# auniquesun/PPT

Measured on AMD Instinct MI355X. Metric: point-clouds/sec fwd+bwd, PointBERT 1024-pt ModelNet40, higher is better.
Workload: dtype f16; 1 GPU; C2: ModelNet40 1024-pt PointBERT (ULIP_PointBERT head_type=0, frozen backbone + PromptLearner), train-mode BN + DropPath, fwd + CE(ls 0.2) + bwd + AdamW; feed=resident, per_gpu_batch=32, global_batch=32, npoints=1024, classes=40, parallelism=dp1

## Files before the change

### include/ppt_hip.h

```cpp
#ifndef PPT_HIP_H
#define PPT_HIP_H

#include <stddef.h>
#include <stdint.h>

#ifdef __cplusplus
extern "C" {
#endif

#define PPT_OK 0
#define PPT_EINVAL (-1)
#define PPT_ELAUNCH (-2)
#define PPT_EUNSUPPORTED (-3)

#define PPT_F32 0
#define PPT_BF16 1
#define PPT_F16 2

const char *ppt_strerror(int code);
int ppt_abi_version(void);

int ppt_fps_f32(const float *xyz, int B, int N, int M, const int64_t *start, int64_t *out_idx,
                float *out_xyz, void *stream);

// ... 181 lines not shown
    int wave_prio;
} ppt_text_lin_params;
int ppt_text_lin_retile_split(const float *W, void *W_tiled, int N, int K, int b_pow2, void *stream);
int ppt_text_lin_split(const ppt_text_lin_params *p, void *stream);
typedef struct ppt_text_lin16_params {
    const void *A; int64_t lda;
    const void *W;
    const float *bias;
    const float *residual; int64_t ld_res;
    void *C; int64_t ldc;
    int M, N, K;
    int dtype;
    int c_dtype;
    int wave_prio;
} ppt_text_lin16_params;
int ppt_text_lin_retile16(const void *W, void *W_tiled, int N, int K, void *stream);
int ppt_text_lin16(const ppt_text_lin16_params *p, void *stream);

int ppt_attention_fwd(const void *qkv, void *out, float *lse, int Bt, int T, int H, int hd,
                      float scale, int causal, int dtype, void *stream);
int ppt_attention_bwd(const void *qkv, const void *out, const void *dout, const float *lse,
                      float *delta, void *dqkv, int Bt, int T, int H, int hd, float scale,
                      int causal, int dtype, void *stream);

size_t ppt_attention_prefix_workspace_bytes(int C, int P, int H, int hd);
int ppt_attention_fwd_split16(const void *qkv, void *out, float *lse, int Bt, int T, int P, int H, int hd, float scale, int causal,
                              void *stream);
int ppt_attention_bwd_split16(const void *qkv, const void *out, const void *dout, const float *lse, float *delta, void *dqkv,
                              float *workspace, int Bt, int T, int P, int H, int hd, float scale, int causal, void *stream);
int ppt_attention_prefix_fwd(const void *qkv, void *out, float *lse, int C, int T, int P, int H, int hd, float scale, int dtype,
                             void *stream);
int ppt_attention_prefix_bwd(const void *qkv, const void *out, const void *dout, const float *lse, float *delta, void *dqkv,
                             float *workspace, int C, int T, int P, int H, int hd, float scale, int dtype, void *stream);

int ppt_conv1_stats(const float *pts, int64_t M, const float *w1, const float *b1, int C,
                    float *part_sum, float *part_sqsum, int *n_partials, void *stream);
int ppt_bn_finalize(const float *part_sum, const float *part_sqsum, int n_partials,
                    int rows_per_partial, int64_t count, int C, const float *gamma, const float *beta, float eps, int train,
                    float momentum, float *running_mean, float *running_var,
                    int64_t *num_batches_tracked, float *scale, float *shift, void *stream);
size_t ppt_bn_finalize_workspace_bytes(int n_partials, int C);
int ppt_bn_finalize_ws(const float *part_sum, const float *part_sqsum, int n_partials,
                       int rows_per_partial, int64_t count, int C, const float *gamma, const float *beta, float eps, int train,
                       float momentum, float *running_mean, float *running_var,
                       int64_t *num_batches_tracked, float *scale, float *shift,
                       float *mean_out , float *rstd_out ,
                       void *workspace, size_t workspace_bytes, void *stream);

int ppt_rows_stats_rows_per_partial(void);
int ppt_rows_stats_f32(const float *x, int64_t M, int C, float *part_sum, float *part_m2, void *stream);
int ppt_bn_rows_bwd_reduce(const float *dy, const float *x, const float *scale, const float *shift, const float *mean,
                           const float *rstd, int relu, int64_t M, int C, float *part_g, float *part_gx, void *stream);
int ppt_bn_rows_bwd_apply(const float *dy, const float *x, const float *scale, const float *shift, const float *mean,
                          const float *rstd, const float *sum_g, const float *sum_gx, int relu, int batch_stats, int64_t M,
                          int C, float *dx, void *dx_half, int half_dtype, void *stream);
int ppt_conv1_stats_max_partials(int64_t M);
int ppt_conv1_stats_rows_per_partial(void);

int ppt_gn_stats_chunks(int R);
int ppt_gn_bwd_chunks(int Q);
int ppt_gn_finish(const double *part, int B, int nch, int G, double n, double eps, int mode, float *out0, float *out1, void *stream);
int ppt_gn_stats(const float *y, int B, int R, int C, int G, double *part, void *stream);
int ppt_gn_lrelu_max(const float *y, const float *mean, const float *rstd, const float *gamma, const float *beta, int B, int Q, int K,
                     int C, int G, float slope, float *out, int32_t *arg, void *stream);
int ppt_gn_bwd_sums(const float *y, const float *dout, const float *out, const int32_t *arg, const float *mean, const float *rstd,
                    const float *gamma, int B, int Q, int K, int C, int G, float slope, double *psum, float *pgb, void *stream);
// ... 114 lines not shown
```

### ppt_amd/_lib.py

```python
import ctypes
import os

_HERE = os.path.dirname(os.path.abspath(__file__))
LIB_PATH = os.environ.get("PPT_HIP_LIB") or os.path.join(_HERE, "csrc", "libppt_hip.so")
_lib = None

PPT_F32, PPT_BF16, PPT_F16 = 0, 1, 2
A_PLAIN, A_AFFINE_RELU, A_CONV1 = 0, 1, 2
ACT_NONE, ACT_RELU, ACT_GELU, ACT_QUICKGELU = 0, 1, 2, 3

c_void_p, c_int, c_int64, c_float, c_size_t = (ctypes.c_void_p, ctypes.c_int, ctypes.c_int64,
                                               ctypes.c_float, ctypes.c_size_t)


class GemmParams(ctypes.Structure):
    _fields_ = [
        ("A", c_void_p), ("lda", c_int64), ("B", c_void_p), ("ldb", c_int64),
        ("C", c_void_p), ("ldc", c_int64), ("M", c_int), ("N", c_int), ("K", c_int),
        ("dtype", c_int), ("c_dtype", c_int),
        ("a_mode", c_int), ("a_scale", c_void_p), ("a_shift", c_void_p), ("pts", c_void_p),
        ("w1", c_void_p), ("b1", c_void_p),
        ("bias", c_void_p), ("group_add", c_void_p), ("group_rows", c_int), ("act", c_int),
        ("dact_pre", c_void_p), ("ld_dact", c_int64),
        ("row_scale", c_void_p), ("row_scale_rows", c_int),
        ("residual", c_void_p), ("ld_res", c_int64), ("residual2", c_void_p), ("ld_res2", c_int64),
        ("C2", c_void_p), ("ldc2", c_int64), ("c2_dtype", c_int), ("c2_pre", c_int),
        ("col_sum", c_void_p), ("col_sqsum", c_void_p), ("pool_max", c_void_p), ("pool_dtype", c_int), ("pool_rows", c_int), ("pool_min", c_void_p),
        ("batch", c_int), ("strideA", c_int64), ("strideB", c_int64), ("strideC", c_int64), ("wave_prio", c_int),
        ("split16", c_int), ("split_a_pow2", c_int), ("split_b_pow2", c_int), ("split_overflow", c_void_p),
    ]


class LnLinParams(ctypes.Structure):
    _fields_ = [
        ("x", c_void_p), ("W", c_void_p), ("C", c_void_p), ("ln_w", c_void_p), ("ln_b", c_void_p), ("ln_eps", ctypes.c_float),
        ("bias", c_void_p), ("M", c_int), ("N", c_int), ("K", c_int), ("dtype", c_int), ("slices", c_int),
    ]


class TextLinParams(ctypes.Structure):
# ... 87 lines not shown
    "ppt_lnlin_retile": (c_int, [c_void_p, c_void_p, c_int, c_void_p]),
    "ppt_lnlin": (c_int, [ctypes.POINTER(LnLinParams), c_void_p]),
    "ppt_text_mlp_retile": (c_int, [c_void_p, c_void_p, c_void_p, c_void_p, c_void_p]),
    "ppt_text_mlp_pair": (c_int, [ctypes.POINTER(TextMlpParams), c_void_p]),
    "ppt_text_mlp_retile_split": (c_int, [c_void_p, c_void_p, c_void_p, c_void_p, c_int, c_void_p]),
    "ppt_text_lin_retile_split": (c_int, [c_void_p, c_void_p, c_int, c_int, c_int, c_void_p]),
    "ppt_text_lin_split": (c_int, [ctypes.POINTER(TextLinParams), c_void_p]),
    "ppt_text_lin_retile16": (c_int, [c_void_p, c_void_p, c_int, c_int, c_void_p]),
    "ppt_text_lin16": (c_int, [ctypes.POINTER(TextLin16Params), c_void_p]),
    "ppt_vit_mlp3_retile": (c_int, [c_void_p, c_void_p, c_void_p, c_void_p, c_void_p]),
    "ppt_vit_mlp3_bf16": (c_int, [ctypes.POINTER(VitMlpParams), c_void_p]),
    "ppt_rowgemm_bf16": (c_int, [ctypes.POINTER(RowGemmParams), c_void_p]),
    "ppt_layernorm_fwd": (c_int, [c_void_p, c_void_p, c_int, c_void_p, c_void_p, c_void_p, c_void_p, c_int,
                                  c_void_p, c_void_p, c_int, c_int, c_float, c_void_p]),
    "ppt_layernorm_bwd": (c_int, [c_void_p, c_void_p, c_void_p, c_void_p, c_void_p, c_void_p, c_int,
                                  c_void_p, c_int, c_void_p, c_void_p, c_int, c_int, c_int, c_void_p]),
    "ppt_layernorm_fwd_sum": (c_int, [c_void_p, c_void_p, c_void_p, c_int, c_void_p, c_void_p, c_void_p, c_void_p, c_int,
                                      c_void_p, c_void_p, c_int, c_int, c_float, c_void_p]),
    "ppt_layernorm_bwd_sum": (c_int, [c_void_p, c_int, c_void_p, c_void_p, c_void_p, c_void_p, c_void_p, c_int,
                                      c_void_p, c_int, c_int, c_int, c_void_p]),
    "ppt_col_sums": (c_int, [c_void_p, c_int, c_int, c_int, c_int64, c_void_p, c_void_p]),
    "ppt_attention_fwd": (c_int, [c_void_p, c_void_p, c_void_p, c_int, c_int, c_int, c_int, c_float, c_int,
                                  c_int, c_void_p]),
    "ppt_attention_bwd": (c_int, [c_void_p, c_void_p, c_void_p, c_void_p, c_void_p, c_void_p, c_int, c_int,
                                  c_int, c_int, c_float, c_int, c_int, c_void_p]),
    "ppt_attention_prefix_workspace_bytes": (ctypes.c_size_t, [c_int, c_int, c_int, c_int]),
    "ppt_pointmlp_cloud_rstd": (c_int, [c_void_p, c_int, c_int, ctypes.c_double, c_void_p, c_void_p]),
    "ppt_pointmlp_pq": (c_int, [c_void_p, c_void_p, c_void_p, c_void_p, c_void_p, c_void_p, c_int, c_int, c_int, c_int, c_void_p]),
    "ppt_attention_bwd_split16": (c_int, [c_void_p, c_void_p, c_void_p, c_void_p, c_void_p, c_void_p, c_void_p, c_int, c_int, c_int, c_int, c_int, c_float, c_int, c_void_p]),
    "ppt_attention_fwd_split16": (c_int, [c_void_p, c_void_p, c_void_p, c_int, c_int, c_int, c_int, c_int, c_float, c_int, c_void_p]),
    "ppt_attention_prefix_fwd": (c_int, [c_void_p, c_void_p, c_void_p, c_int, c_int, c_int, c_int, c_int, c_float, c_int, c_void_p]),
    "ppt_attention_prefix_bwd": (c_int, [c_void_p, c_void_p, c_void_p, c_void_p, c_void_p, c_void_p, c_void_p, c_int, c_int, c_int,
                                         c_int, c_int, c_float, c_int, c_void_p]),
    "ppt_conv1_stats": (c_int, [c_void_p, c_int64, c_void_p, c_void_p, c_int, c_void_p, c_void_p,
                                ctypes.POINTER(c_int), c_void_p]),
    "ppt_conv1_stats_max_partials": (c_int, [c_int64]),
    "ppt_conv1_stats_rows_per_partial": (c_int, []),
    "ppt_bn_finalize": (c_int, [c_void_p, c_void_p, c_int, c_int, c_int64, c_int, c_void_p, c_void_p, c_float, c_int,
                                c_float, c_void_p, c_void_p, c_void_p, c_void_p, c_void_p, c_void_p]),
    "ppt_bn_finalize_ws": (c_int, [c_void_p, c_void_p, c_int, c_int, c_int64, c_int, c_void_p, c_void_p, c_float, c_int,
                                   c_float, c_void_p, c_void_p, c_void_p, c_void_p, c_void_p, c_void_p, c_void_p, c_void_p,
                                   ctypes.c_size_t, c_void_p]),
    "ppt_rows_stats_rows_per_partial": (c_int, []),
    "ppt_rows_stats_f32": (c_int, [c_void_p, c_int64, c_int, c_void_p, c_void_p, c_void_p]),
    "ppt_bn_rows_bwd_reduce": (c_int, [c_void_p, c_void_p, c_void_p, c_void_p, c_void_p, c_void_p, c_int, c_int64, c_int,
                                       c_void_p, c_void_p, c_void_p]),
    "ppt_bn_rows_bwd_apply": (c_int, [c_void_p, c_void_p, c_void_p, c_void_p, c_void_p, c_void_p, c_void_p, c_void_p, c_int,
                                      c_int, c_int64, c_int, c_void_p, c_void_p, c_int, c_void_p]),
    "ppt_bn_finalize_workspace_bytes": (ctypes.c_size_t, [c_int, c_int]),
    "ppt_gn_stats_chunks": (c_int, [c_int]),
    "ppt_gn_bwd_chunks": (c_int, [c_int]),
    "ppt_gn_stats": (c_int, [c_void_p, c_int, c_int, c_int, c_int, c_void_p, c_void_p]),
    "ppt_gn_lrelu_max": (c_int, [c_void_p, c_void_p, c_void_p, c_void_p, c_void_p, c_int, c_int, c_int, c_int, c_int, c_float,
                                 c_void_p, c_void_p, c_void_p]),
    "ppt_gn_bwd_sums": (c_int, [c_void_p, c_void_p, c_void_p, c_void_p, c_void_p, c_void_p, c_void_p, c_int, c_int, c_int, c_int,
                                c_int, c_float, c_void_p, c_void_p, c_void_p]),
    "ppt_gn_bwd_apply": (c_int, [c_void_p, c_void_p, c_void_p, c_void_p, c_void_p, c_void_p, c_void_p, c_void_p, c_int, c_int,
                                 c_int, c_int, c_int, c_float, c_void_p, c_void_p]),
    "ppt_mini_pointnet_conv12_bf16": (c_int, [c_void_p, c_int64, c_void_p, c_void_p, c_void_p, c_void_p, c_int, c_void_p, c_void_p,
                                              c_int, c_void_p, c_void_p, c_void_p]),
    "ppt_mini_pointnet_conv3_bf16": (c_int, [c_void_p, c_int64, c_int, c_void_p, c_void_p, c_int, c_void_p, c_void_p, c_void_p,
                                             c_void_p]),
    "ppt_mini_pointnet_conv4_bf16": (c_int, [c_void_p, c_int64, c_int, c_void_p, c_void_p, c_void_p, c_void_p, c_int, c_void_p,
                                             c_void_p]),
    "ppt_mini_pointnet_conv12_half": (c_int, [c_void_p, c_int64, c_void_p, c_void_p, c_void_p, c_void_p, c_int, c_void_p, c_void_p,
                                              c_int, c_void_p, c_void_p, c_int, c_void_p]),
# ... 61 lines not shown
```

### ppt_amd/csrc/attention.hip

```cpp
#include "attn_common.h"

namespace {

constexpr int SEG = 16, KT = 32, ROWS = 64;

__device__ __forceinline__ float quad_sum(float v)
{
    v += __uint_as_float(dpp_mov<0xB1, 0xf>(__float_as_uint(v)));
    v += __uint_as_float(dpp_mov<0x4E, 0xf>(__float_as_uint(v)));
    return v;
}

template <typename T>
__device__ __forceinline__ void stage_rows(const T *__restrict__ base, int64_t row_stride, int r0, int Tlen,
                                           float *dst, int Tfull, int P, int v)
{
    for (int i = threadIdx.x; i < KT * HD; i += blockDim.x) {
        const int r = i >> 6, d = i & 63;
        dst[i] = (r0 + r) < Tlen ? dt<T>::load(base + am_row(Tfull, P, v, r0 + r) * row_stride + d) : 0.0f;
    }
}

template <typename T>
__global__ __launch_bounds__(256) void attn_fwd_quad(const T *__restrict__ qkv, T *__restrict__ out,
// ... 334 lines not shown
        if (rc != PPT_EUNSUPPORTED) return rc;
        return f16 ? attn_bwd_t<f16_t>(qkv, out, dout, lse, delta, dqkv, Bt, T, H, scale, causal, P, part, false, s)
                   : attn_bwd_t<bf16_t>(qkv, out, dout, lse, delta, dqkv, Bt, T, H, scale, causal, P, part, false, s);
    }
    return PPT_EINVAL;
}

extern "C" int ppt_attention_bwd(const void *qkv, const void *out, const void *dout, const float *lse, float *delta,
                                 void *dqkv, int Bt, int T, int H, int hd, float scale, int causal, int dtype,
                                 void *stream)
{
    return attn_bwd_any(qkv, out, dout, lse, delta, dqkv, nullptr, Bt, T, 0, H, hd, scale, causal, dtype, stream);
}

extern "C" size_t ppt_attention_prefix_workspace_bytes(int C, int P, int H, int hd)
{
    return (size_t)(C + 1) * (size_t)P * 2 * (size_t)H * (size_t)hd * sizeof(float);
}

extern "C" int ppt_attention_prefix_fwd(const void *qkv, void *out, float *lse, int C, int T, int P, int H, int hd, float scale,
                                        int dtype, void *stream)
{
    if (P <= 0 || P >= T) return PPT_EINVAL;
    return attn_fwd_any(qkv, out, lse, C, T, P, H, hd, scale, 1, dtype, stream);
}

extern "C" int ppt_attention_prefix_bwd(const void *qkv, const void *out, const void *dout, const float *lse, float *delta,
                                        void *dqkv, float *part, int C, int T, int P, int H, int hd, float scale, int dtype,
                                        void *stream)
{
    if (P <= 0 || P >= T) return PPT_EINVAL;
    return attn_bwd_any(qkv, out, dout, lse, delta, dqkv, part, C, T, P, H, hd, scale, 1, dtype, stream);
}
```

### ppt_amd/csrc/attention_mfma.hip

```cpp
#include <stdlib.h>
#include <type_traits>
#include "attn_common.h"

namespace {

template <int FORM> struct AttnForm {
    using F = typename std::conditional<FORM == PPT_BF16, bf16_t, f16_t>::type;
    using T = bf16_t;
    using chunk_t = uint4;
    static constexpr int IMAGES = 1, CH_SHIFT = 3;
    static constexpr float P_PRE = 1.0f;
    struct Q { chunk_t raw[4][1]; };

    static __device__ __forceinline__ chunk_t zero() { return make_uint4(0, 0, 0, 0); }
    static __device__ __forceinline__ void prep_q(Q &, int) {}
    static __device__ __forceinline__ void write(unsigned char *kimg, unsigned char *vimg, int row, int ch, const chunk_t &k, const chunk_t &v)
    {
        *reinterpret_cast<uint4 *>(kimg + k_off(row, ch)) = k;
        *reinterpret_cast<uint4 *>(vimg + v_off(row, ch * 16)) = v;
    }
    static __device__ __forceinline__ float peel_dot(const T *kl, const Q &q, int h)
    {
        float dot = 0.f;
#pragma unroll
// ... 878 lines not shown
__global__ __launch_bounds__(256, 2) void attn_bwd_dq_mfma(const bf16_t *__restrict__ qkv, const bf16_t *__restrict__ dout,
                                                        const float *__restrict__ lse, const float *__restrict__ delta,
                                                        bf16_t *__restrict__ dqkv, int Tfull, int H, float scale, int P, int C)
{
    __shared__ __align__(16) unsigned char smem[DQ_SMEM];
    attn_bwd_dq_body<F, CAUSAL, false>(qkv, nullptr, dout, lse, delta, dqkv, Tfull, H, scale, P, C, smem, blockIdx.x, blockIdx.y);
}

#ifndef PPT_SHORT_OCC
#define PPT_SHORT_OCC 2
#endif
template <bool CAUSAL, typename F>
__global__ __launch_bounds__(256, PPT_SHORT_OCC) void attn_bwd_short_mfma(const bf16_t *__restrict__ qkv, const bf16_t *__restrict__ out,
                                                           const bf16_t *__restrict__ dout, const float *__restrict__ lse,
                                                           bf16_t *__restrict__ dqkv, int Tfull, int H, float scale, int P, int C,
                                                           float *__restrict__ part, int prio)
{
    PPT_PRIO(prio);
    __shared__ __align__(16) unsigned char smem[DQ_SMEM > DKV_SMEM ? DQ_SMEM : DKV_SMEM];
#ifdef PPT_SHORT_ROLE
    if (PPT_SHORT_ROLE == 0) { attn_bwd_dkv_body<F, CAUSAL, true, false>(qkv, out, dout, lse, nullptr, dqkv, Tfull, H, scale, P, C, part, smem, 0, blockIdx.y); return; }
    if (PPT_SHORT_ROLE == 1) { attn_bwd_dq_body<F, CAUSAL, true>(qkv, out, dout, lse, nullptr, dqkv, Tfull, H, scale, P, C, smem, 0, blockIdx.y); return; }
    if (PPT_SHORT_ROLE == 2) return;
#endif
    if (gridDim.x == 1 || blockIdx.x == 0)
        attn_bwd_dkv_body<F, CAUSAL, true, false>(qkv, out, dout, lse, nullptr, dqkv, Tfull, H, scale, P, C, part, smem, 0, blockIdx.y);
    if (gridDim.x == 1) __syncthreads();
    if (gridDim.x == 1 || blockIdx.x == 1)
        attn_bwd_dq_body<F, CAUSAL, true>(qkv, out, dout, lse, nullptr, dqkv, Tfull, H, scale, P, C, smem, 0, blockIdx.y);
}


constexpr int TINY_SMEM = 7 * TILE + 512;
template <bool CAUSAL, typename F>
__global__ __launch_bounds__(256, 2) void attn_bwd_tiny_mfma(const bf16_t *__restrict__ qkv, const bf16_t *__restrict__ out,
                                                          const bf16_t *__restrict__ dout, const float *__restrict__ lse,
                                                          bf16_t *__restrict__ dqkv, int Tfull, int H, float scale, int P, int C,
                                                          float *__restrict__ part, int prio)
{
    PPT_PRIO(prio);
    __shared__ __align__(16) unsigned char smem[TINY_SMEM];
    unsigned char *Qr = smem, *Qt = smem + TILE, *Gr = smem + 2 * TILE, *Gt = smem + 3 * TILE, *Kr = smem + 4 * TILE, *Kt = smem + 5 * TILE,
                  *Vr = smem + 6 * TILE;
    float *L2 = reinterpret_cast<float *>(smem + 7 * TILE), *DL = L2 + 64;
    const int lane = threadIdx.x & 63;
    const int w = __builtin_amdgcn_readfirstlane(threadIdx.x >> 6);
    const int r = lane & 31, h = lane >> 5;
    const int bh = blockIdx.y, b = bh / H, head = bh % H;
    const int64_t rs = 3 * (int64_t)H * HD, os = (int64_t)H * HD;
    const int T = am_len(Tfull, P, C, b), q_lo = am_qlo(P, C, b);
    const float c = scale * 1.4426950408889634f;

    {
        uint4 q[2], k[2], v[2], g[2];
        float dl[2], l2[2];
#pragma unroll
        for (int i = 0; i < 2; ++i) {
            const int row = 32 * i + (threadIdx.x >> 3), ch = threadIdx.x & 7;
            q[i] = k[i] = v[i] = g[i] = make_uint4(0, 0, 0, 0);
            uint4 o = make_uint4(0, 0, 0, 0);
            l2[i] = INFINITY;
            const bool own = row < T && row >= q_lo;
            if (row < T) {
                const int64_t pr = am_row(Tfull, P, b, row);
                const bf16_t *qp = qkv + pr * rs + head * HD + ch * 8;
                q[i] = *reinterpret_cast<const uint4 *>(qp);
                k[i] = *reinterpret_cast<const uint4 *>(qp + H * HD);
                v[i] = *reinterpret_cast<const uint4 *>(qp + 2 * H * HD);
                g[i] = *reinterpret_cast<const uint4 *>(dout + pr * os + head * HD + ch * 8);
                o = *reinterpret_cast<const uint4 *>(out + pr * os + head * HD + ch * 8);
                if (own && ch == 0) l2[i] = lse[am_stat(Tfull, P, H, b, head, row)] * 1.4426950408889634f;
            }
            float d = dot8_bf16<F>(g[i], o);
            d += __shfl_xor(d, 1); d += __shfl_xor(d, 2); d += __shfl_xor(d, 4);
            dl[i] = own ? d : 0.f;
        }
#pragma unroll
        for (int i = 0; i < 2; ++i) {
            const int row = 32 * i + (threadIdx.x >> 3), ch = threadIdx.x & 7;
            *reinterpret_cast<uint4 *>(Qr + k_off(row, ch)) = q[i];
            *reinterpret_cast<uint4 *>(Qt + v_off(row, ch * 16)) = q[i];
            *reinterpret_cast<uint4 *>(Gr + k_off(row, ch)) = g[i];
            *reinterpret_cast<uint4 *>(Gt + v_off(row, ch * 16)) = g[i];
            *reinterpret_cast<uint4 *>(Kr + k_off(row, ch)) = k[i];
            *reinterpret_cast<uint4 *>(Kt + v_off(row, ch * 16)) = k[i];
            *reinterpret_cast<uint4 *>(Vr + k_off(row, ch)) = v[i];
// ... 190 lines not shown
        PPT_CHECK_LAUNCH();
        return PPT_OK;
    }
    return ppt_attention_fwd_stream(qkv, out, lse, Bt, T, H, scale, causal, P, fmt, s);
}

extern "C" int ppt_attention_bwd_short_mfma_bf16(const void *qkv, const void *out, const void *dout, const float *lse, void *dqkv, int Bt, int T,
                                                 int H, float scale, int causal, int P, float *part, int fmt, hipStream_t s)
{
    if (T > 128) return PPT_EUNSUPPORTED;
    if (((uintptr_t)qkv & 15) || ((uintptr_t)out & 15) || ((uintptr_t)dout & 15) || ((uintptr_t)dqkv & 7) || ((uintptr_t)part & 15)) return PPT_EUNSUPPORTED;
    static const int both = [] { const char *e = getenv("PPT_ATTN_SHORT_BOTH"); return e ? atoi(e) : 1; }();
    static const int tiny = [] { const char *e = getenv("PPT_ATTN_TINY"); return e ? atoi(e) : 1; }();
    const int pairs = (Bt + (P > 0)) * H;
    if (tiny && T <= 64 && !((uintptr_t)dout & 15)) {
        const int prio = ppt_get_wave_priority();
#define PPT_LAUNCH_TINY(CA, TT) hipLaunchKernelGGL((attn_bwd_tiny_mfma<CA, TT>), dim3(1, pairs), dim3(256), 0, s, (const bf16_t *)qkv, (const bf16_t *)out, (const bf16_t *)dout, lse, (bf16_t *)dqkv, T, H, scale, P, Bt, part, prio)
        if (fmt == PPT_F16) { if (causal) PPT_LAUNCH_TINY(true, f16_t); else PPT_LAUNCH_TINY(false, f16_t); }
        else { if (causal) PPT_LAUNCH_TINY(true, bf16_t); else PPT_LAUNCH_TINY(false, bf16_t); }
#undef PPT_LAUNCH_TINY
        PPT_CHECK_LAUNCH();
        return PPT_OK;
    }
    dim3 grid(both && 2 * pairs > 512 ? 1 : 2, pairs);
    const int prio = ppt_get_wave_priority();
#define PPT_LAUNCH_SHORT(CA, TT) hipLaunchKernelGGL((attn_bwd_short_mfma<CA, TT>), grid, dim3(256), 0, s, (const bf16_t *)qkv, (const bf16_t *)out, (const bf16_t *)dout, lse, (bf16_t *)dqkv, T, H, scale, P, Bt, part, prio)
    if (fmt == PPT_F16) { if (causal) PPT_LAUNCH_SHORT(true, f16_t); else PPT_LAUNCH_SHORT(false, f16_t); }
    else { if (causal) PPT_LAUNCH_SHORT(true, bf16_t); else PPT_LAUNCH_SHORT(false, bf16_t); }
#undef PPT_LAUNCH_SHORT
    PPT_CHECK_LAUNCH();
    return PPT_OK;
}

extern "C" int ppt_attention_bwd_mfma_bf16(const void *qkv, const void *dout, const float *lse, const float *delta,
                                           void *dqkv, int Bt, int T, int H, float scale, int causal, int P, float *part,
                                           int fmt, hipStream_t s)
{
    if (((uintptr_t)qkv & 15) || ((uintptr_t)dout & 15) || ((uintptr_t)dqkv & 7) || ((uintptr_t)part & 15)) return PPT_EUNSUPPORTED;
    dim3 grid((T + 127) / 128, (Bt + (P > 0)) * H);
#define PPT_LAUNCH_BWD(CA, TT) do { \
        hipLaunchKernelGGL((attn_bwd_dkv_mfma<CA, TT>), grid, dim3(256), 0, s, (const bf16_t *)qkv, (const bf16_t *)dout, lse, delta, (bf16_t *)dqkv, T, H, scale, P, Bt, part); \
        hipLaunchKernelGGL((attn_bwd_dq_mfma<CA, TT>), grid, dim3(256), 0, s, (const bf16_t *)qkv, (const bf16_t *)dout, lse, delta, (bf16_t *)dqkv, T, H, scale, P, Bt); } while (0)
    if (fmt == PPT_F16) { if (causal) PPT_LAUNCH_BWD(true, f16_t); else PPT_LAUNCH_BWD(false, f16_t); }
    else { if (causal) PPT_LAUNCH_BWD(true, bf16_t); else PPT_LAUNCH_BWD(false, bf16_t); }
#undef PPT_LAUNCH_BWD
    PPT_CHECK_LAUNCH();
    return PPT_OK;
}
```

### ppt_amd/csrc/attn_common.h

```cpp
#pragma once
#include "ppt_common.h"
#include "attn_rowmap.h"

typedef __attribute__((ext_vector_type(4))) short s4_t;
typedef __attribute__((ext_vector_type(16))) float f32x16_t;

constexpr int HD = 64, KVT = 64, QB = 128, TILE = KVT * 128;
constexpr int QT = 32, QTILE = QT * 128;

__device__ __forceinline__ int k_off(int row, int chunk) { return row * 128 + ((chunk ^ ((row >> 1) & 7)) << 4); }
__device__ __forceinline__ int v_off(int key, int dbyte) { return key * 128 + (dbyte ^ (((key >> 1) & 1) << 6)); }

__device__ __forceinline__ uint4 tr_frag(const unsigned char *img, int row0, int dbyte)
{
    struct { s4_t a, b; } f;
    f.a = __builtin_amdgcn_ds_read_tr16_b64_v4i16((__attribute__((address_space(3))) s4_t *)(img + v_off(row0, dbyte)));
    f.b = __builtin_amdgcn_ds_read_tr16_b64_v4i16((__attribute__((address_space(3))) s4_t *)(img + v_off(row0 + 8, dbyte)));
    return __builtin_bit_cast(uint4, f);
}

__device__ __forceinline__ void attn_xcd_map(int xcd_map, int &qblk, int &bh)
{
    bh = blockIdx.y, qblk = blockIdx.x;
    if (xcd_map && (gridDim.y & 7) == 0) {
// ... 16 lines not shown
{
    const _Float16 ha = (_Float16)a, hb = (_Float16)b;
    const h2_t hh = {ha, hb};
    const h2_t ll = {(_Float16)(a - (float)ha), (_Float16)(b - (float)hb)};
    hi = __builtin_bit_cast(uint32_t, hh);
    lo = __builtin_bit_cast(uint32_t, ll);
}
__device__ __forceinline__ void split8(const float4 &u, const float4 &v, uint4 &hi, uint4 &lo)
{
    split2(u.x, u.y, hi.x, lo.x); split2(u.z, u.w, hi.y, lo.y);
    split2(v.x, v.y, hi.z, lo.z); split2(v.z, v.w, hi.w, lo.w);
}
__device__ __forceinline__ f32x16_t mfma3(uint4 ah, uint4 al, uint4 bh, uint4 bl, f32x16_t c)
{
    c = h16<f16_t>::mfma32(al, bh, c);
    c = h16<f16_t>::mfma32(ah, bl, c);
    return h16<f16_t>::mfma32(ah, bh, c);
}
__device__ __forceinline__ void split_acc(const f32x16_t &x, int s, uint4 &hi, uint4 &lo)
{
    split2(x[8 * s + 0], x[8 * s + 1], hi.x, lo.x); split2(x[8 * s + 2], x[8 * s + 3], hi.y, lo.y);
    split2(x[8 * s + 4], x[8 * s + 5], hi.z, lo.z); split2(x[8 * s + 6], x[8 * s + 7], hi.w, lo.w);
}

extern "C" {
int ppt_attention_fwd_stream(const void *qkv, void *out, float *lse, int Bt, int T, int H, float scale, int causal, int P, int form,
                             hipStream_t s);
int ppt_attention_fwd_mfma_bf16(const void *qkv, void *out, float *lse, int Bt, int T, int H, float scale, int causal, int P, int fmt,
                                hipStream_t s);
int ppt_attention_bwd_mfma_bf16(const void *qkv, const void *dout, const float *lse, const float *delta, void *dqkv, int Bt, int T,
                                int H, float scale, int causal, int P, float *part, int fmt, hipStream_t s);
int ppt_attention_bwd_short_mfma_bf16(const void *qkv, const void *out, const void *dout, const float *lse, void *dqkv, int Bt, int T,
                                      int H, float scale, int causal, int P, float *part, int fmt, hipStream_t s);
int ppt_attention_fwd_quad_bf16(const void *qkv, void *out, float *lse, int Bt, int T, int H, float scale, int causal, int P, int fmt,
                                hipStream_t s);
int ppt_attention_prefix_reduce_f32(const float *part, void *dqkv, int Bt, int P, int H, int prio, hipStream_t s);
}
```

### ppt_amd/engine.py

```python
import os

import torch

from . import ops
from .ops import ACT_GELU, ACT_NONE, ACT_QUICKGELU, A_AFFINE_RELU, A_CONV1

ATTN_SCALE = 64 ** -0.5


class WeightCache:

    def __init__(self, dtype, demoted=None):
        self.dtype = dtype
        self._c = {}
        self.demoted = demoted if demoted is not None else set()

    def get(self, t, kind="w", cols=None, pad_to=None):
        key = (id(t), kind, cols, pad_to)
        ent = self._c.get(key)
        if ent is not None and ent[0] is t and ent[1] == t._version:
            return ent[2]
        with torch.no_grad():
            w = t.detach()
            w = w.reshape(w.shape[0], -1)
# ... 650 lines not shown
        for j in range(nb):
            y = _mlp_res_block(sd, wc, f"{pp}operation.{j}.", y, train, upd, pool=k if j == nb - 1 else 1,
                               x_affine=aff if j == 0 else None)
        nb = cfg["pos_blocks"][i]
        for j in range(nb):
            y = _mlp_res_block(sd, wc, f"{p}pos_blocks_list.{i}.operation.{j}.", y, train, upd,
                               pool=S if (i == n_stage - 1 and j == nb - 1) else 1)
        x, xyz, N = y, new_xyz, S
    c = p + "classifier."
    for fc, bn, mask in (("0.", "1.", 0), ("4.", "5.", 1)):
        w = wc.get(sd[c + fc + "weight"])
        st = _stats_bufs(B, w.shape[0], dev, train)
        h = ops.gemm(x, w, out_dtype=torch.float32, bias=sd[c + fc + "bias"], col_stats=st)
        sc, sh = _bn_affine(sd, c + bn, train, st, 32, B, upd)
        last = fc == "4."
        x = ops.bn_act_rows(h, sc, sh, torch.float32 if last else T, mask=drop_masks[mask] if drop_masks is not None else None)
    return x


TEXT_FUSE_LN = os.environ.get("PPT_TEXT_FUSE_LN", "0") != "0"
TEXT_SPLITK = os.environ.get("PPT_TEXT_SPLITK", "1") != "0"
POINTMLP_FUSED_NORM = os.environ.get("PPT_POINTMLP_FUSED_NORM", "1") != "0"


TEXT_MLP_PAIR = os.environ.get("PPT_TEXT_MLP_PAIR", "1") != "0"
TEXT_MLP_PAIR_LN = os.environ.get("PPT_TEXT_MLP_PAIR_LN", "1") != "0"
TEXT_MLP_PAIR_LAST = os.environ.get("PPT_TEXT_MLP_PAIR_LAST", "1") != "0"
TEXT_MLP_PAIR_SPLIT = os.environ.get("PPT_TEXT_MLP_PAIR_SPLIT", "1") != "0"


TEXT_LIN_SPLIT = os.environ.get("PPT_TEXT_LIN_SPLIT", "1") != "0"


def _text_lin_ok(Ta, width):
    return TEXT_LIN_SPLIT and width == 512 and (Ta in ops.HALF or (Ta == torch.float32 and ops.split16_enabled()))


def _text_lin_tiles(sd, name, wca, transposed=False):
    w = sd[name]
    if wca.dtype in ops.HALF:
        return wca.derived(("text_lin16", name, transposed), (w,),
                           lambda: ops.text_lin_retile16(wca.get(w, "wt") if transposed else wca.get(w)))
    b = ops.SPLIT16_POW2[1]
    return wca.derived(("text_lin_split", name, transposed, b), (w,),
                       lambda: ops.text_lin_retile_split(wca.get(w, "wt") if transposed else wca.get(w), b))


def _text_lin(a, sd, name, wca, transposed=False, **kw):
    wt = _text_lin_tiles(sd, name, wca, transposed)
    return ops.text_lin16(a, wt, **kw) if wca.dtype in ops.HALF else ops.text_lin_split(a, wt, **kw)


def _text_mlp_pair_ok(Tm):
    return Tm in ops.HALF or (Tm == torch.float32 and TEXT_MLP_PAIR_SPLIT and ops.split16_enabled())


def _text_mlp_tiles(sd, p, wcm, backward):
    wfc, wpr = sd[p + "mlp.c_fc.weight"], sd[p + "mlp.c_proj.weight"]
    b = ops.SPLIT16_POW2[1] if wcm.dtype == torch.float32 else None
    if backward:
        return wcm.derived(("text_mlp_tiles_bwd", p, b), (wfc, wpr), lambda: ops.text_mlp_retile(wcm.get(wpr, "wt"), wcm.get(wfc, "wt"), b))
    return wcm.derived(("text_mlp_tiles_fwd", p, b), (wfc, wpr), lambda: ops.text_mlp_retile(wcm.get(wfc), wcm.get(wpr), b))


def _text_mlp(a, sd, p, wcm, *, pre=None, backward=False, save=False):
    w1t, w2t = _text_mlp_tiles(sd, p, wcm, backward)
# ... 127 lines not shown
        out = ops.gemm(hn, wc32.get(sd["text_projection"], "wt"), out_dtype=torch.float32)
    if save:
        saved.update(x_eot=x_eot, meanf=meanf, rstdf=rstdf, rows=rows, C=C, L=L, Lfull=Lfull, W=Wd, heads=heads, P=P, M=M,
                     rows_mode=rows_in is not None, wca=wca, wcm=wcm)
    return out, saved


_F32_CACHES = {}


def _f32_cache(wc):
    c = _F32_CACHES.get(id(wc))
    if c is None or c[0] is not wc:
        c = (wc, WeightCache(torch.float32))
        _F32_CACHES[id(wc)] = c
    return c[1]


def text_tower_backward(sd, wc, s, dout, grad_scale=1.0):
    T = wc.dtype
    S = float(grad_scale)
    C, L, Wd, heads, P, M = s["C"], s["L"], s["W"], s["heads"], s["P"], s["M"]
    wc32 = _f32_cache(wc)
    d_hn = ops.rows_matmul(dout.contiguous(), wc32.get(sd["text_projection"], "wt"), alpha=S) if dout.shape[0] <= 256 else None
    if d_hn is None:
        d_hn = ops.gemm(dout.contiguous() if S == 1.0 else dout * S, wc32.get(sd["text_projection"], "w"), out_dtype=torch.float32)
    d_eot, _, _ = ops.layernorm_bwd(d_hn, s["x_eot"], sd["ln_final.weight"], s["meanf"], s["rstdf"])
    g = torch.zeros((M, Wd), dtype=torch.float32, device=dout.device)
    g.index_copy_(0, s["rows"], d_eot)
    wca, wcm = s.get("wca", wc), s.get("wcm", wc)
    Ta, Tm = wca.dtype, wcm.dtype
    splitk = TEXT_SPLITK and (T in ops.HALF or ops.split16_enabled()) and Ta == T and Tm == T and M <= 4096 and Wd == 512
    lin_split = _text_lin_ok(Ta, Wd) and splitk and Tm == Ta
    g_t = ops.convert(g, Tm)
    for i in reversed(range(len(s["layers"]))):
        p = f"transformer.resblocks.{i}."
        ly = s["layers"][i]
        if TEXT_MLP_PAIR and splitk and _text_mlp_pair_ok(Tm) and tuple(sd[p + "mlp.c_fc.weight"].shape) == (2048, 512):
            _, g_t = ops.layernorm_bwd_sum(_text_mlp(g_t, sd, p, wcm, pre=ly["pre"], backward=True), ly["x_mid"],
                                           sd[p + "ln_2.weight"], ly["mean2"], ly["rstd2"], g, accumulate=True, copy_dtype=Ta)
            d_pre = None
        else:
            d_pre = ops.gemm(g_t, wcm.get(sd[p + "mlp.c_proj.weight"], "wt"), out_dtype=Tm, act=ACT_QUICKGELU,
                             dact_pre=ly["pre"])
        if d_pre is None:
            pass
        elif splitk:
            _, g_t = ops.layernorm_bwd_sum(ops.gemm_splitk(d_pre, wcm.get(sd[p + "mlp.c_fc.weight"], "wt"), 4), ly["x_mid"],
                                           sd[p + "ln_2.weight"], ly["mean2"], ly["rstd2"], g, accumulate=True, copy_dtype=Ta)
        else:
            d_h2 = ops.gemm(d_pre, wcm.get(sd[p + "mlp.c_fc.weight"], "wt"), out_dtype=torch.float32)
            _, _, _, g_t = ops.layernorm_bwd(d_h2, ly["x_mid"], sd[p + "ln_2.weight"], ly["mean2"], ly["rstd2"], dx=g,
                                             accumulate=True, copy_dtype=Ta)
        if lin_split:
            d_a = _text_lin(g_t, sd, p + "attn.out_proj.weight", wca, True)
        else:
            d_a = ops.gemm(g_t, wca.get(sd[p + "attn.out_proj.weight"], "wt"), out_dtype=Ta)
        if P:
            d_qkv = ops.attention_prefix_bwd(ly["qkv"], ly["a"], d_a, ly["lse"], C, L, P, heads, ATTN_SCALE)
        else:
            d_qkv = ops.attention_bwd(ly["qkv"], ly["a"], d_a, ly["lse"], C, L, heads, ATTN_SCALE, True)
        if splitk:
            dparts = (_text_lin(d_qkv, sd, p + "attn.in_proj_weight", wca, True) if lin_split
                      else ops.gemm_splitk(d_qkv, wca.get(sd[p + "attn.in_proj_weight"], "wt"), 3))
            _, g_t = ops.layernorm_bwd_sum(dparts, ly["x"],
                                           sd[p + "ln_1.weight"], ly["mean1"], ly["rstd1"], g, accumulate=True, copy_dtype=Tm)
        else:
            d_h = ops.gemm(d_qkv, wca.get(sd[p + "attn.in_proj_weight"], "wt"), out_dtype=torch.float32)
            _, _, _, g_t = ops.layernorm_bwd(d_h, ly["x"], sd[p + "ln_1.weight"], ly["mean1"], ly["rstd1"], dx=g,
                                             accumulate=True, copy_dtype=Tm)
    if s["rows_mode"]:
        return g
    if S != 1.0:
        g.mul_(1.0 / S)
    if not P and L == s["Lfull"]:
        return g.view(C, L, Wd)
    full = torch.zeros((C, s["Lfull"], Wd), dtype=torch.float32, device=dout.device)
    if P:
        full[0, :P] = g[:P]
        full[:, P:L] = g[P:].view(C, L - P, Wd)
    else:
        full[:, :L] = g.view(C, L, Wd)
    return full


def head_loss_forward_backward(feat, wt, text_raw, logit_scale, labels, smoothing, w=None):
    B, C = feat.shape[0], text_raw.shape[0]
    if w is not None and w.dtype == torch.float32 and feat.shape[1] <= 8192 and B <= 4096 and logit_scale.dtype == torch.float32:
        return ops.head_loss(feat.contiguous(), w.contiguous(), text_raw.contiguous(), logit_scale.contiguous(),
                             labels.contiguous(), smoothing)
    pc = ops.gemm(feat.contiguous(), wt, out_dtype=torch.float32, split=False)
    nrm = text_raw.norm(dim=-1, keepdim=True)
    tn = text_raw / nrm
    spc = (logit_scale.exp() * pc).contiguous()
# ... 11 lines not shown
```

### ppt_amd/ops.py

```python
import ctypes
import os

import torch

from . import _lib
from ._lib import (ACT_GELU, ACT_NONE, ACT_QUICKGELU, ACT_RELU, A_AFFINE_RELU, A_CONV1, A_PLAIN,
                   PPT_BF16, PPT_F16, PPT_F32, GemmParams, RowGemmParams)
from . import _lib as _libmod

_DT = {torch.float32: PPT_F32, torch.bfloat16: PPT_BF16, torch.float16: PPT_F16}
_TORCH_DT = {PPT_F32: torch.float32, PPT_BF16: torch.bfloat16, PPT_F16: torch.float16}
HALF = (torch.bfloat16, torch.float16)


class KernelProfiler:

    def __init__(self):
        self.records = []
        self.kernels = []
        self.executed = []

    def begin(self, name, work, kernel=None, executed=None):
        ev = torch.cuda.Event(enable_timing=True)
        ev.record(torch.cuda.current_stream())
# ... 660 lines not shown
        _lib.check(L.ppt_attention_bwd_split16(_p(qkv), _p(out), _p(dout), _p(lse), _p(delta), _p(dqkv), _p(ws), n_seq, T, P, H, 64,
                                               scale, int(causal), _stream()), "ppt_attention_bwd_split16")
    elif P:
        _lib.check(L.ppt_attention_prefix_bwd(_p(qkv), _p(out), _p(dout), _p(lse), _p(delta), _p(dqkv), _p(ws), n_seq, T, P, H, 64,
                                              scale, dtype_code(qkv), _stream()), "ppt_attention_prefix_bwd")
    else:
        _lib.check(L.ppt_attention_bwd(_p(qkv), _p(out), _p(dout), _p(lse), _p(delta), _p(dqkv), n_seq, T, H, 64,
                                       scale, int(causal), dtype_code(qkv), _stream()), "ppt_attention_bwd")
    if profiler is not None:
        profiler.end()
    return dqkv


def attention_fwd(qkv, Bt, T, H, scale, causal, want_lse=True):
    return _attention_fwd(qkv, Bt, T, 0, H, scale, causal, want_lse)


def attention_bwd(qkv, out, dout, lse, Bt, T, H, scale, causal):
    return _attention_bwd(qkv, out, dout, lse, Bt, T, 0, H, scale, causal)


def prefix_rows(C, T, P):
    return P + C * (T - P)


def attention_prefix_fwd(qkv, C, T, P, H, scale, want_lse=True):
    return _attention_fwd(qkv, C, T, P, H, scale, True, want_lse)


def attention_prefix_bwd(qkv, out, dout, lse, C, T, P, H, scale):
    return _attention_bwd(qkv, out, dout, lse, C, T, P, H, scale, True)


def conv1_stats(pts, w1, b1):
    _chk(pts, torch.float32, "pts")
    M = pts.shape[0]
    C = w1.shape[0]
    P = _lib.lib().ppt_conv1_stats_max_partials(M)
    ps = torch.empty((P, C), dtype=torch.float32, device=pts.device)
    pq = torch.empty((P, C), dtype=torch.float32, device=pts.device)
    n = ctypes.c_int(0)
    _lib.check(_lib.lib().ppt_conv1_stats(_p(pts), M, _p(w1), _p(b1), C, _p(ps), _p(pq), ctypes.byref(n), _stream()),
               "ppt_conv1_stats")
    return ps, pq, _lib.lib().ppt_conv1_stats_rows_per_partial()


def bn_finalize(gamma, beta, train, partials=None, rows_per_partial=0, count=0, running_mean=None, running_var=None,
                num_batches_tracked=None, eps=1e-5, momentum=0.1, update_running=True, want_moments=False):
    C = gamma.shape[0]
    mean = torch.empty((C,), dtype=torch.float32, device=gamma.device) if want_moments else None
    rstd = torch.empty((C,), dtype=torch.float32, device=gamma.device) if want_moments else None
    scale = torch.empty((C,), dtype=torch.float32, device=gamma.device)
    shift = torch.empty((C,), dtype=torch.float32, device=gamma.device)
    ps, pq = partials if partials is not None else (None, None)
    upd = train and update_running
    P = 0 if ps is None else ps.shape[0]
    wbytes = _lib.lib().ppt_bn_finalize_workspace_bytes(P, C) if train else 0
    ws = torch.empty((wbytes // 8,), dtype=torch.float64, device=gamma.device) if wbytes else None
    _lib.check(_lib.lib().ppt_bn_finalize_ws(_p(ps), _p(pq), P, rows_per_partial, count, C, _p(gamma),
                                             _p(beta), eps, int(train), momentum,
                                             _p(running_mean) if (upd or not train) else None,
                                             _p(running_var) if (upd or not train) else None,
                                             _p(num_batches_tracked) if upd else None, _p(scale), _p(shift), _p(mean), _p(rstd),
                                             _p(ws), wbytes, _stream()),
               "ppt_bn_finalize_ws")
    return (scale, shift, mean, rstd) if want_moments else (scale, shift)
# ... 542 lines not shown
```

Measured before the change: 12480 point-clouds/s.

## Fuse out_proj backward GEMM into tiny prefix attention backward kernel

Adds a fused variant of the tiny MFMA attention-backward kernel that computes d_out = g·W_out for its head directly from pre-tiled out_proj weights in shared memory and feeds it to the attention backward. The text-encoder backward loop uses it by default when the shapes fit (prefix P, L<=64, 8 heads, half dtype), and falls back to the separate GEMM plus attention kernel when the fused kernel reports unsupported. This removes one kernel launch and the global round-trip of d_a per layer. In exchange, each attention block repeats the per-head GEMM work and uses a larger shared-memory footprint, which may lower occupancy.

```diff
diff --git a/include/ppt_hip.h b/include/ppt_hip.h
--- a/include/ppt_hip.h
+++ b/include/ppt_hip.h
@@ -237,6 +237,9 @@
                              void *stream);
 int ppt_attention_prefix_bwd(const void *qkv, const void *out, const void *dout, const float *lse, float *delta, void *dqkv,
                              float *workspace, int C, int T, int P, int H, int hd, float scale, int dtype, void *stream);
+int ppt_attention_prefix_bwd_fused(const void *qkv, const void *out, const void *g, const void *wout_tiles, const float *lse,
+                                   void *dqkv, float *workspace, void *dout_dump, int C, int T, int P, int H, int hd, float scale,
+                                   int dtype, void *stream);
 
 int ppt_conv1_stats(const float *pts, int64_t M, const float *w1, const float *b1, int C,
                     float *part_sum, float *part_sqsum, int *n_partials, void *stream);
diff --git a/ppt_amd/_lib.py b/ppt_amd/_lib.py
--- a/ppt_amd/_lib.py
+++ b/ppt_amd/_lib.py
@@ -6,6 +6,7 @@
 _lib = None
 
 PPT_F32, PPT_BF16, PPT_F16 = 0, 1, 2
+PPT_EUNSUPPORTED = -3
 A_PLAIN, A_AFFINE_RELU, A_CONV1 = 0, 1, 2
 ACT_NONE, ACT_RELU, ACT_GELU, ACT_QUICKGELU = 0, 1, 2, 3
 
@@ -159,6 +160,8 @@
     "ppt_attention_prefix_fwd": (c_int, [c_void_p, c_void_p, c_void_p, c_int, c_int, c_int, c_int, c_int, c_float, c_int, c_void_p]),
     "ppt_attention_prefix_bwd": (c_int, [c_void_p, c_void_p, c_void_p, c_void_p, c_void_p, c_void_p, c_void_p, c_int, c_int, c_int,
                                          c_int, c_int, c_float, c_int, c_void_p]),
+    "ppt_attention_prefix_bwd_fused": (c_int, [c_void_p, c_void_p, c_void_p, c_void_p, c_void_p, c_void_p, c_void_p, c_void_p, c_int, c_int,
+                                               c_int, c_int, c_int, c_float, c_int, c_void_p]),
     "ppt_conv1_stats": (c_int, [c_void_p, c_int64, c_void_p, c_void_p, c_int, c_void_p, c_void_p,
                                 ctypes.POINTER(c_int), c_void_p]),
     "ppt_conv1_stats_max_partials": (c_int, [c_int64]),
diff --git a/ppt_amd/csrc/attention.hip b/ppt_amd/csrc/attention.hip
--- a/ppt_amd/csrc/attention.hip
+++ b/ppt_amd/csrc/attention.hip
@@ -390,3 +390,16 @@
     if (P <= 0 || P >= T) return PPT_EINVAL;
     return attn_bwd_any(qkv, out, dout, lse, delta, dqkv, part, C, T, P, H, hd, scale, 1, dtype, stream);
 }
+
+extern "C" int ppt_attention_prefix_bwd_fused(const void *qkv, const void *out, const void *g, const void *wout_tiles, const float *lse,
+                                              void *dqkv, float *part, void *dout_dump, int C, int T, int P, int H, int hd, float scale,
+                                              int dtype, void *stream)
+{
+    if (!qkv || !out || !g || !wout_tiles || !lse || !dqkv || !part || C <= 0 || T <= 0 || P <= 0 || P >= T) return PPT_EINVAL;
+    if (hd != HD || (dtype != PPT_BF16 && dtype != PPT_F16)) return PPT_EUNSUPPORTED;
+    hipStream_t s = ppt_stream(stream);
+    const int rc = ppt_attention_bwd_tiny_fused_bf16(qkv, out, g, wout_tiles, lse, dqkv, dout_dump, C, T, H, scale, P, part, dtype, s);
+    if (rc != PPT_OK) return rc;
+    const int prio = ppt_get_wave_priority();
+    return dtype == PPT_F16 ? attn_reduce_t<f16_t>(part, dqkv, C, P, H, prio, s) : attn_reduce_t<bf16_t>(part, dqkv, C, P, H, prio, s);
+}
diff --git a/ppt_amd/csrc/attention_mfma.hip b/ppt_amd/csrc/attention_mfma.hip
--- a/ppt_amd/csrc/attention_mfma.hip
+++ b/ppt_amd/csrc/attention_mfma.hip
@@ -934,14 +934,17 @@
 
 
 constexpr int TINY_SMEM = 7 * TILE + 512;
-template <bool CAUSAL, typename F>
+constexpr int FUSE_AP = 2 * 512 + 32;
+constexpr int FUSE_SMEM = 64 * FUSE_AP > TINY_SMEM ? 64 * FUSE_AP : TINY_SMEM;
+template <bool CAUSAL, typename F, bool FUSE_OUT = false>
 __global__ __launch_bounds__(256, 2) void attn_bwd_tiny_mfma(const bf16_t *__restrict__ qkv, const bf16_t *__restrict__ out,
                                                           const bf16_t *__restrict__ dout, const float *__restrict__ lse,
                                                           bf16_t *__restrict__ dqkv, int Tfull, int H, float scale, int P, int C,
-                                                          float *__restrict__ part, int prio)
+                                                          float *__restrict__ part, int prio,
+                                                          const unsigned char *__restrict__ wout = nullptr, bf16_t *__restrict__ do_dump = nullptr)
 {
     PPT_PRIO(prio);
-    __shared__ __align__(16) unsigned char smem[TINY_SMEM];
+    __shared__ __align__(16) unsigned char smem[FUSE_OUT ? FUSE_SMEM : TINY_SMEM];
     unsigned char *Qr = smem, *Qt = smem + TILE, *Gr = smem + 2 * TILE, *Gt = smem + 3 * TILE, *Kr = smem + 4 * TILE, *Kt = smem + 5 * TILE,
                   *Vr = smem + 6 * TILE;
     float *L2 = reinterpret_cast<float *>(smem + 7 * TILE), *DL = L2 + 64;
@@ -953,7 +956,100 @@
     const int T = am_len(Tfull, P, C, b), q_lo = am_qlo(P, C, b);
     const float c = scale * 1.4426950408889634f;
 
-    {
+    if constexpr (FUSE_OUT) {
+        const int n_own = T - q_lo;
+        const bool wide = n_own > 32;
+        uint4 gv[4][4];
+#pragma unroll
+        for (int rb = 0; rb < 4; ++rb)
+#pragma unroll
+            for (int it = 0; it < 4; ++it) {
+                const int lr = 16 * rb + 4 * it + w;
+                gv[rb][it] = make_uint4(0, 0, 0, 0);
+                if (lr < n_own) gv[rb][it] = *reinterpret_cast<const uint4 *>(dout + am_row(Tfull, P, b, q_lo + lr) * os + 8 * lane);
+            }
+        uint4 q[2], k[2], v[2], o[2];
+        float l2[2];
+#pragma unroll
+        for (int i = 0; i < 2; ++i) {
+            const int row = 32 * i + (threadIdx.x >> 3), ch = threadIdx.x & 7;
+            q[i] = k[i] = v[i] = o[i] = make_uint4(0, 0, 0, 0);
+            l2[i] = INFINITY;
+            if (row < T) {
+                const int64_t pr = am_row(Tfull, P, b, row);
+                const bf16_t *qp = qkv + pr * rs + head * HD + ch * 8;
+                q[i] = *reinterpret_cast<const uint4 *>(qp);
+                k[i] = *reinterpret_cast<const uint4 *>(qp + H * HD);
+                v[i] = *reinterpret_cast<const uint4 *>(qp + 2 * H * HD);
+                o[i] = *reinterpret_cast<const uint4 *>(out + pr * os + head * HD + ch * 8);
+                if (row >= q_lo && ch == 0) l2[i] = lse[am_stat(Tfull, P, H, b, head, row)] * 1.4426950408889634f;
+            }
+        }
+        constexpr int D1 = 8, K1 = 16;
+        const unsigned char *wp = wout + (size_t)((4 * head + w) * K1) * 1024 + lane * 16;
+        uint4 ring[D1];
+#pragma unroll
+        for (int i = 0; i < D1; ++i) ring[i] = *reinterpret_cast<const uint4 *>(wp + 1024 * i);
+#pragma unroll
+        for (int rb = 0; rb < 4; ++rb)
+            if (rb < 2 || wide)
+#pragma unroll
+                for (int it = 0; it < 4; ++it)
+                    *reinterpret_cast<uint4 *>(smem + (16 * rb + 4 * it + w) * FUSE_AP + 16 * lane) = gv[rb][it];
+        __syncthreads();
+
+        const int l15 = lane & 15, kg = lane >> 4;
+        ppt_f32x4 acc[4];
+#pragma unroll
+        for (int rb = 0; rb < 4; ++rb) acc[rb] = ppt_f32x4{0.f, 0.f, 0.f, 0.f};
+        const unsigned char *ha = smem + l15 * FUSE_AP + 16 * kg;
+#pragma unroll
+        for (int ks = 0; ks < K1; ++ks) {
+            const uint4 f0 = *reinterpret_cast<const uint4 *>(ha + 64 * ks), f1 = *reinterpret_cast<const uint4 *>(ha + 16 * FUSE_AP + 64 * ks);
+            acc[0] = h16<F>::mfma16(ring[ks % D1], f0, acc[0]);
+            acc[1] = h16<F>::mfma16(ring[ks % D1], f1, acc[1]);
+            if (wide) {
+                const uint4 f2 = *reinterpret_cast<const uint4 *>(ha + 32 * FUSE_AP + 64 * ks), f3 = *reinterpret_cast<const uint4 *>(ha + 48 * FUSE_AP + 64 * ks);
+                acc[2] = h16<F>::mfma16(ring[ks % D1], f2, acc[2]);
+                acc[3] = h16<F>::mfma16(ring[ks % D1], f3, acc[3]);
+            }
+            if (ks + D1 < K1) ring[ks % D1] = *reinterpret_cast<const uint4 *>(wp + 1024 * (ks + D1));
+        }
+        __syncthreads();
+
+#pragma unroll
+        for (int rb = 0; rb < 4; ++rb) {
+            const int lr = 16 * rb + l15, row = q_lo + lr, col = 16 * w + 4 * kg;
+            if (lr < n_own) {
+                const uint2 u = make_uint2(h16<F>::pack2(acc[rb][0], acc[rb][1]), h16<F>::pack2(acc[rb][2], acc[rb][3]));
+                *reinterpret_cast<uint2 *>(Gr + k_off(row, col >> 3) + 2 * (col & 7)) = u;
+                *reinterpret_cast<uint2 *>(Gt + v_off(row, 2 * col)) = u;
+                if (do_dump) *reinterpret_cast<uint2 *>(do_dump + am_row(Tfull, P, b, row) * os + head * HD + col) = u;
+            }
+        }
+#pragma unroll
+        for (int i = 0; i < 2; ++i) {
+            const int row = 32 * i + (threadIdx.x >> 3), ch = threadIdx.x & 7;
+            *reinterpret_cast<uint4 *>(Qr + k_off(row, ch)) = q[i];
+            *reinterpret_cast<uint4 *>(Qt + v_off(row, ch * 16)) = q[i];
+            *reinterpret_cast<uint4 *>(Kr + k_off(row, ch)) = k[i];
+            *reinterpret_cast<uint4 *>(Kt + v_off(row, ch * 16)) = k[i];
+            *reinterpret_cast<uint4 *>(Vr + k_off(row, ch)) = v[i];
+            if (row >= T || row < q_lo) {
+                *reinterpret_cast<uint4 *>(Gr + k_off(row, ch)) = make_uint4(0, 0, 0, 0);
+                *reinterpret_cast<uint4 *>(Gt + v_off(row, ch * 16)) = make_uint4(0, 0, 0, 0);
+            }
+            if (ch == 0) L2[row] = l2[i];
+        }
+        __syncthreads();
+#pragma unroll
+        for (int i = 0; i < 2; ++i) {
+            const int row = 32 * i + (threadIdx.x >> 3), ch = threadIdx.x & 7;
+            float d = dot8_bf16<F>(*reinterpret_cast<const uint4 *>(Gr + k_off(row, ch)), o[i]);
+            d += __shfl_xor(d, 1); d += __shfl_xor(d, 2); d += __shfl_xor(d, 4);
+            if (ch == 0) DL[row] = (row < T && row >= q_lo) ? d : 0.f;
+        }
+    } else {
         uint4 q[2], k[2], v[2], g[2];
         float dl[2], l2[2];
 #pragma unroll
@@ -1210,6 +1306,20 @@
     return PPT_OK;
 }
 
+extern "C" int ppt_attention_bwd_tiny_fused_bf16(const void *qkv, const void *out, const void *g, const void *wout, const float *lse, void *dqkv,
+                                                 void *do_dump, int Bt, int T, int H, float scale, int P, float *part, int fmt, hipStream_t s)
+{
+    if (T > 64 || H != 8 || P <= 0 || P >= T) return PPT_EUNSUPPORTED;
+    if (((uintptr_t)qkv & 15) || ((uintptr_t)out & 15) || ((uintptr_t)g & 15) || ((uintptr_t)wout & 15) || ((uintptr_t)dqkv & 7) ||
+        ((uintptr_t)part & 15) || ((uintptr_t)do_dump & 7)) return PPT_EUNSUPPORTED;
+    const int pairs = (Bt + 1) * H, prio = ppt_get_wave_priority();
+#define PPT_LAUNCH_TINY_FUSED(TT) hipLaunchKernelGGL((attn_bwd_tiny_mfma<true, TT, true>), dim3(1, pairs), dim3(256), 0, s, (const bf16_t *)qkv, (const bf16_t *)out, (const bf16_t *)g, lse, (bf16_t *)dqkv, T, H, scale, P, Bt, part, prio, (const unsigned char *)wout, (bf16_t *)do_dump)
+    if (fmt == PPT_F16) PPT_LAUNCH_TINY_FUSED(f16_t); else PPT_LAUNCH_TINY_FUSED(bf16_t);
+#undef PPT_LAUNCH_TINY_FUSED
+    PPT_CHECK_LAUNCH();
+    return PPT_OK;
+}
+
 extern "C" int ppt_attention_bwd_mfma_bf16(const void *qkv, const void *dout, const float *lse, const float *delta,
                                            void *dqkv, int Bt, int T, int H, float scale, int causal, int P, float *part,
                                            int fmt, hipStream_t s)
diff --git a/ppt_amd/csrc/attn_common.h b/ppt_amd/csrc/attn_common.h
--- a/ppt_amd/csrc/attn_common.h
+++ b/ppt_amd/csrc/attn_common.h
@@ -72,6 +72,8 @@
                                 int H, float scale, int causal, int P, float *part, int fmt, hipStream_t s);
 int ppt_attention_bwd_short_mfma_bf16(const void *qkv, const void *out, const void *dout, const float *lse, void *dqkv, int Bt, int T,
                                       int H, float scale, int causal, int P, float *part, int fmt, hipStream_t s);
+int ppt_attention_bwd_tiny_fused_bf16(const void *qkv, const void *out, const void *g, const void *wout, const float *lse, void *dqkv,
+                                      void *do_dump, int Bt, int T, int H, float scale, int P, float *part, int fmt, hipStream_t s);
 int ppt_attention_fwd_quad_bf16(const void *qkv, void *out, float *lse, int Bt, int T, int H, float scale, int causal, int P, int fmt,
                                 hipStream_t s);
 int ppt_attention_prefix_reduce_f32(const float *part, void *dqkv, int Bt, int P, int H, int prio, hipStream_t s);
diff --git a/ppt_amd/engine.py b/ppt_amd/engine.py
--- a/ppt_amd/engine.py
+++ b/ppt_amd/engine.py
@@ -706,6 +706,9 @@
 TEXT_LIN_SPLIT = os.environ.get("PPT_TEXT_LIN_SPLIT", "1") != "0"
 
 
+TEXT_ATTN_BWD_FUSE_OUT = os.environ.get("PPT_TEXT_ATTN_BWD_FUSE_OUT", "1") != "0"
+
+
 def _text_lin_ok(Ta, width):
     return TEXT_LIN_SPLIT and width == 512 and (Ta in ops.HALF or (Ta == torch.float32 and ops.split16_enabled()))
 
@@ -899,6 +902,7 @@
     Ta, Tm = wca.dtype, wcm.dtype
     splitk = TEXT_SPLITK and (T in ops.HALF or ops.split16_enabled()) and Ta == T and Tm == T and M <= 4096 and Wd == 512
     lin_split = _text_lin_ok(Ta, Wd) and splitk and Tm == Ta
+    fuse_out = TEXT_ATTN_BWD_FUSE_OUT and lin_split and Ta in ops.HALF and P and L <= 64 and heads == 8
     g_t = ops.convert(g, Tm)
     for i in reversed(range(len(s["layers"]))):
         p = f"transformer.resblocks.{i}."
@@ -919,14 +923,17 @@
             d_h2 = ops.gemm(d_pre, wcm.get(sd[p + "mlp.c_fc.weight"], "wt"), out_dtype=torch.float32)
             _, _, _, g_t = ops.layernorm_bwd(d_h2, ly["x_mid"], sd[p + "ln_2.weight"], ly["mean2"], ly["rstd2"], dx=g,
                                              accumulate=True, copy_dtype=Ta)
-        if lin_split:
-            d_a = _text_lin(g_t, sd, p + "attn.out_proj.weight", wca, True)
-        else:
-            d_a = ops.gemm(g_t, wca.get(sd[p + "attn.out_proj.weight"], "wt"), out_dtype=Ta)
-        if P:
-            d_qkv = ops.attention_prefix_bwd(ly["qkv"], ly["a"], d_a, ly["lse"], C, L, P, heads, ATTN_SCALE)
-        else:
-            d_qkv = ops.attention_bwd(ly["qkv"], ly["a"], d_a, ly["lse"], C, L, heads, ATTN_SCALE, True)
+        d_qkv = ops.attention_prefix_bwd_fused(ly["qkv"], ly["a"], g_t, _text_lin_tiles(sd, p + "attn.out_proj.weight", wca, True),
+                                               ly["lse"], C, L, P, heads, ATTN_SCALE) if fuse_out else None
+        if d_qkv is None:
+            if lin_split:
+                d_a = _text_lin(g_t, sd, p + "attn.out_proj.weight", wca, True)
+            else:
+                d_a = ops.gemm(g_t, wca.get(sd[p + "attn.out_proj.weight"], "wt"), out_dtype=Ta)
+            if P:
+                d_qkv = ops.attention_prefix_bwd(ly["qkv"], ly["a"], d_a, ly["lse"], C, L, P, heads, ATTN_SCALE)
+            else:
+                d_qkv = ops.attention_bwd(ly["qkv"], ly["a"], d_a, ly["lse"], C, L, heads, ATTN_SCALE, True)
         if splitk:
             dparts = (_text_lin(d_qkv, sd, p + "attn.in_proj_weight", wca, True) if lin_split
                       else ops.gemm_splitk(d_qkv, wca.get(sd[p + "attn.in_proj_weight"], "wt"), 3))
diff --git a/ppt_amd/ops.py b/ppt_amd/ops.py
--- a/ppt_amd/ops.py
+++ b/ppt_amd/ops.py
@@ -716,6 +716,27 @@
     return _attention_bwd(qkv, out, dout, lse, C, T, P, H, scale, True)
 
 
+def attention_prefix_bwd_fused(qkv, out, g, wout_t, lse, C, T, P, H, scale, dout_dump=None):
+    rows = prefix_rows(C, T, P)
+    assert qkv.dim() == 2 and qkv.shape[0] == rows and g.shape == (rows, H * 64) and g.is_contiguous() and qkv.is_contiguous()
+    assert out.dtype == qkv.dtype and g.dtype == qkv.dtype and out.is_contiguous() and lse.dtype == torch.float32
+    assert wout_t.dtype == torch.uint8 and wout_t.numel() == 2 * 512 * 512
+    assert dout_dump is None or (dout_dump.shape == g.shape and dout_dump.dtype == qkv.dtype and dout_dump.is_contiguous())
+    dqkv = torch.empty_like(qkv)
+    L = _lib.lib()
+    ws = torch.empty((L.ppt_attention_prefix_workspace_bytes(C, P, H, 64) // 4,), dtype=torch.float32, device=qkv.device)
+    if profiler is not None:
+        profiler.begin("attention_bwd", 5.0 * _attn_pairs(C, T, P, True) * H * 64 + 2.0 * rows * (H * 64) ** 2)
+    rc = L.ppt_attention_prefix_bwd_fused(_p(qkv), _p(out), _p(g), _p(wout_t), _p(lse), _p(dqkv), _p(ws), _p(dout_dump), C, T, P, H, 64,
+                                          scale, dtype_code(qkv), _stream())
+    if profiler is not None:
+        profiler.end()
+    if rc == _lib.PPT_EUNSUPPORTED:
+        return None
+    _lib.check(rc, "ppt_attention_prefix_bwd_fused")
+    return dqkv
+
+
 def conv1_stats(pts, w1, b1):
     _chk(pts, torch.float32, "pts")
     M = pts.shape[0]
```

Result: no change. 12500 point-clouds/s (median of 6 runs) (+0.1%).
